# Da-Tsuchi/KLab_MultiModalModel

Measured on AMD Instinct MI355X. Metric: caption-train samples/sec (224px img, 64-tok tgt), higher is better.
Workload: dtype bf16; 1 GPU; BASELINE configs[1]: Swin-V2(C=64,(2,2,6,2),224,w7) frozen + T5-small, fwd+bwd+Adam, T5 dropout 0.1 on, random-init weights; global_batch=64, per_gpu_batch=64, src_len=9, tgt_len=64, parallelism=dp1, hipgraph=False, optimizer=klab.optim.FusedAdam (Adam update of ref/train.py:28, one kernel)

## Files before the change

### include/klab_mm.h

```cpp
#ifndef KLAB_MM_H
#define KLAB_MM_H
#include <stddef.h>
#include <stdint.h>

#ifdef __cplusplus
extern "C" {
#endif

#define KLAB_OK 0
#define KLAB_ERR_UNSUPPORTED (-2)
#define KLAB_ERR_BADARG (-3)

#define KLAB_F32 0
#define KLAB_BF16 1
#define KLAB_FP8 2

#define KLAB_ACT_NONE 0
#define KLAB_ACT_RELU 1
#define KLAB_ACT_GELU 2

#define KLAB_AUX_NONE 0
#define KLAB_AUX_NONZERO 1
#define KLAB_AUX_DGELU 2

// ... 77 lines not shown
int klab_t5_attn_fwd(const klab_attn_args* a, void* stream);
int klab_t5_attn_bwd(const klab_attn_args* a, void* stream);
typedef struct klab_attn_fused_args {
  const float* x; const float* gamma; float eps; int d_model;
  const void* w;
  void* xn; float* rstd;
  void* proj; long ldproj;
  int cross;
  klab_attn_args attn;
} klab_attn_fused_args;
int klab_t5_attn_fused_fwd(const klab_attn_fused_args* a, void* stream);
typedef struct klab_attn_bwd_fused_args {
  const void* dy; long lddy;
  const void* w;
  int d_model;
  klab_attn_args attn;
} klab_attn_bwd_fused_args;
int klab_t5_attn_bwd_fused(const klab_attn_bwd_fused_args* a, void* stream);
int klab_dbias_reduce(const void* ds_ws, int dtype, float* dbias, int nbatch, int H, int Lq, int Lk, void* stream);

typedef struct klab_swin_attn_args {
  int dtype;
  const void* qkv; void* ctx; const float* bias; const float* logit_scale; float* lse;
  int B, R, w, shift, H, C;
  const void* dctx; void* dqkv; float* dbias; float* dlogit_scale;
  void* bwd_ws; size_t bwd_ws_bytes;
  const float* bias_table; float* dbias_table;
  const float* v_bias; float* dv_bias;
} klab_swin_attn_args;
int klab_swin_attn_fwd(const klab_swin_attn_args* a, void* stream);
size_t klab_swin_attn_bwd_ws_bytes(int dtype, int B, int R, int w, int H, int C);
int klab_swin_qkv_attn_fused(const void* x, const void* wqkv, const float* bqkv, void* ctx, const float* bias, const float* logit_scale,
                             int dtype, int B, int R, int w, int shift, int H, int C, void* stream);
int klab_swin_attn_bwd(const klab_swin_attn_args* a, void* stream);
int klab_swin_cpb_bias(const float* coords, const int* index, const float* w0, const float* b0, const float* w2,
                       float* table, float* hidden, float* bias, int ntab, int n, int heads, int nhidden, void* stream);
int klab_swin_cpb_table(const float* coords, const float* w0, const float* b0, const float* w2, float* table, float* hidden,
                        float* bias_table, int ntab, int heads, int nhidden, void* stream);
int klab_swin_cpb_table_bwd(const float* dbias_table, const float* bias_table, const float* coords, const float* hidden, const float* w2,
                            float* dtable, float* dw0, float* db0, float* dw2, int ntab, int heads, int nhidden, void* stream);

typedef struct klab_image_desc { long long offset; int height, width; } klab_image_desc;
size_t klab_image_preprocess_ws_bytes(int n_images, int max_h, int mid);
int klab_image_preprocess(const unsigned char* src, const klab_image_desc* desc_dev, int n_images, int max_h, int max_w, int mid,
                          int out_size, int filter_a, int filter_b, double rescale, const float* mean3, const float* std3,
                          float* pixel_values, void* ws, size_t ws_bytes, void* stream);

#define KLAB_JPEG_GRAY 0
#define KLAB_JPEG_YCC 1
#define KLAB_JPEG_RGB 2
typedef struct klab_jpeg_info {
  int width, height, ncomp, precision, progressive, supported, colour;
  int hmax, vmax, mcus_x, mcus_y;
  int hs[3], vs[3], bw[3], bh[3], tq[3];
  long long coef_blocks;
} klab_jpeg_info;
typedef struct klab_jpeg_item { klab_jpeg_info info; long long coef_block0; long long rgb_off; } klab_jpeg_item;
int klab_jpeg_read_info(const unsigned char* data, size_t n, klab_jpeg_info* info);
int klab_jpeg_entropy_decode(const unsigned char* data, size_t n, short* coefs, unsigned short* qt, klab_jpeg_info* info);
int klab_jpeg_entropy_decode_batch(const unsigned char* const* data, const size_t* sizes, int n, short* const* coefs,
                                   unsigned short* qt, klab_jpeg_info* infos, int* rcs, int n_threads);
size_t klab_jpeg_decode_ws_bytes(const klab_jpeg_item* items, int n);
int klab_jpeg_decode_device(const short* coefs_dev, const unsigned short* qt_dev, const klab_jpeg_item* items,
                            const klab_jpeg_item* items_dev, int n, unsigned char* rgb_dev, void* ws, size_t ws_bytes, void* stream);

int klab_cast_pack(const void* desc_dev, int ndesc, long total4, void* dst, int dtype, void* stream);
// ... 204 lines not shown
```

### klab_multimodalmodel_amd/_lib.py

```python
import ctypes as C
import os

HERE = os.path.dirname(os.path.abspath(__file__))
LIB_PATH = os.environ.get("KLAB_LIB", os.path.join(HERE, "libklab_mm.so"))

F32, BF16, FP8 = 0, 1, 2
ACT_NONE, ACT_RELU, ACT_GELU = 0, 1, 2
AUX_NONE, AUX_NONZERO, AUX_DGELU = 0, 1, 2
ERR_UNSUPPORTED, ERR_BADARG = -2, -3

vp, i32, i64, f32, u32 = C.c_void_p, C.c_int, C.c_long, C.c_float, C.c_uint32


class GemmArgs(C.Structure):
    _fields_ = [("M", i32), ("N", i32), ("K", i32), ("dtype", i32),
                ("A", vp), ("lda", i64), ("a_kmajor", i32),
                ("B", vp), ("ldb", i64), ("b_kmajor", i32),
                ("C", vp), ("ldc", i64), ("c_dtype", i32), ("accumulate", i32),
                ("alpha", f32), ("alpha_dev", vp), ("bias", vp), ("act", i32),
                ("aux", vp), ("ldaux", i64), ("aux_mode", i32), ("aux_scale", f32),
                ("residual", vp), ("ldr", i64), ("r_dtype", i32),
                ("drop_p", f32), ("seed_dev", vp), ("drop_tag", u32), ("name_tag", i32), ("atomic_ok", i32)]


# ... 79 lines not shown
    "klab_layernorm_fwd": [vp, i32, vp, vp, vp, vp, vp, i32, vp, vp, i32, i32, f32, i32, i32, i32, f32, vp, u32, vp],
    "klab_layernorm_bwd": [vp, vp, i32, vp, vp, vp, vp, vp, vp, i32, i32, i32, i32, i32, f32, vp, u32, vp],
    "klab_rmsnorm_fwd_q8": [vp, vp, vp, vp, vp, vp, i32, i32, f32, f32, vp, u32, vp],
    "klab_layernorm_fwd_q8": [vp, vp, vp, vp, vp, vp, vp, vp, vp, vp, i32, i32, f32, vp],
    "klab_gelu_fwd": [vp, vp, i32, i64, vp],
    "klab_gelu_fwd_q8": [vp, vp, vp, vp, i32, i32, vp],
    "klab_geglu_fwd": [vp, i64, vp, i64, i32, i32, i32, f32, vp, u32, vp],
    "klab_geglu_bwd": [vp, i64, vp, i64, vp, i64, i32, i32, i32, f32, vp, u32, vp],
    "klab_layernorm_bwd_bias": [vp, vp, i32, vp, vp, vp, vp, vp, vp, vp, i32, i32, i32, i32, i32, f32, vp, u32, vp],
    "klab_t5_attn_fwd": [C.POINTER(AttnArgs), vp],
    "klab_t5_attn_bwd": [C.POINTER(AttnArgs), vp],
    "klab_t5_attn_fused_fwd": [C.POINTER(AttnFusedArgs), vp],
    "klab_t5_attn_bwd_fused": [C.POINTER(AttnBwdFusedArgs), vp],
    "klab_t5_beam_decode_attn": [i32, vp, i64, vp, vp, i64, i64, i32, vp, i64, vp, i64, vp, i64, i32, i32, i32, i32, vp],
    "klab_beam_topk": [i32, vp, i64, i32, vp, i32, i32, i32, vp, vp, vp, vp, vp],
    "klab_beam_update": [C.POINTER(BeamUpdateArgs), i32, vp],
    "klab_beam_init": [C.POINTER(BeamUpdateArgs), i32, i32, vp],
    "klab_beam_copy_rows": [i32, vp, i64, i32, vp, i64, i32, i32, vp],
    "klab_sample_rows": [C.POINTER(SampleArgs), vp],
    "klab_logits_process_rows": [C.POINTER(LogitsProcArgs), vp],
    "klab_gen_finalize": [vp, i64, vp, i64, i32, i32, i32, i32, f32, i32, vp, vp, vp, vp],
    "klab_sizeof_sample_args": [],
    "klab_sizeof_logits_proc_args": [],
    "klab_sizeof_gen_cfg": [],
    "klab_beam_topk_scores": [vp, i64, i32, vp, i32, i32, i32, vp, vp, vp, vp, vp],
    "klab_dbias_reduce": [vp, i32, vp, i32, i32, i32, i32, vp],
    "klab_swin_mlp_fused": [vp, vp, vp, vp, vp, vp, vp, vp, vp, vp, i32, i32, i32, f32, vp],
    "klab_gemm_grouped": [vp, i32, vp],
    "klab_gemm_grouped_tiles": [vp, i32, i32, vp],
    "klab_gemm_fp8": [C.POINTER(GemmArgs), vp, vp, i64, vp],
    "klab_quant_fp8_rows": [vp, i64, i32, i32, vp, i64, vp, vp],
    "klab_quant_fp8_arena": [vp, i32, i64, vp, vp, vp, vp],
    "klab_swin_qkv_attn_fused": [vp, vp, vp, vp, vp, vp, i32, i32, i32, i32, i32, i32, i32, vp],
    "klab_swin_linear_ln_fused": [vp, vp, vp, vp, vp, vp, vp, vp, i32, i32, i32, i32, f32, vp],
    "klab_swin_patch_embed_fused": [vp, vp, i32, vp, vp, vp, vp, vp, i32, i32, i32, i32, i32, i32, f32, vp],
    "klab_swin_proj_ln_fused": [vp, vp, vp, vp, vp, vp, vp, vp, i32, i32, i32, f32, vp],
    "klab_swin_attn_fwd": [C.POINTER(SwinAttnArgs), vp],
    "klab_swin_attn_bwd": [C.POINTER(SwinAttnArgs), vp],
    "klab_swin_attn_bwd_ws_bytes": [i32, i32, i32, i32, i32, i32],
    "klab_swin_cpb_bias": [vp, vp, vp, vp, vp, vp, vp, vp, i32, i32, i32, i32, vp],
    "klab_swin_cpb_table": [vp, vp, vp, vp, vp, vp, vp, i32, i32, i32, vp],
    "klab_swin_cpb_table_bwd": [vp, vp, vp, vp, vp, vp, vp, vp, vp, i32, i32, i32, vp],
    "klab_cast_pack": [vp, i32, i64, vp, i32, vp],
    "klab_embed_fwd": [vp, i32, i32, i32, i32, vp, i32, vp, i32, i32, f32, vp, u32, vp, vp],
    "klab_embed_bwd": [vp, i32, i32, i32, i32, vp, vp, i32, i32, i32, f32, vp, u32, vp],
    "klab_relbias_fwd": [vp, vp, vp, i32, i32, i32, vp],
    "klab_relbias_bwd": [vp, vp, vp, i32, i32, i32, i32, vp],
    "klab_ce_fwd": [vp, i64, i32, vp, i32, i32, vp, vp, vp, i32, vp],
    "klab_ce_count": [vp, i32, vp, vp],
    "klab_im2col_patch": [vp, vp, i32, i32, i32, i32, i32, vp],
    "klab_im2col_patch_ld": [vp, vp, i32, i32, i32, i32, i32, i32, vp],
    "klab_merge_gather": [vp, vp, i32, i32, i32, i32, vp],
    "klab_merge_scatter": [vp, vp, i32, i32, i32, vp],
    "klab_colsum": [vp, i64, i32, i32, i32, vp, vp],
    "klab_convert": [vp, vp, i32, i64, f32, vp],
    "klab_add_f32": [vp, vp, i64, vp],
    "klab_image_preprocess_ws_bytes": [i32, i32, i32],
    "klab_segv_trace_install": [i32],
    "klab_segv_set_context": [C.c_char_p],
    "klab_image_preprocess": [vp, vp, i32, i32, i32, i32, i32, i32, i32, C.c_double, vp, vp, vp, vp, C.c_size_t, vp],
    "klab_jpeg_read_info": [vp, C.c_size_t, vp],
    "klab_jpeg_entropy_decode": [vp, C.c_size_t, vp, vp, vp],
    "klab_jpeg_entropy_decode_batch": [vp, vp, i32, vp, vp, vp, vp, i32],
    "klab_jpeg_decode_ws_bytes": [vp, i32],
    "klab_jpeg_decode_device": [vp, vp, vp, vp, i32, vp, vp, C.c_size_t, vp],
}


class JpegInfo(C.Structure):
    _fields_ = [("width", i32), ("height", i32), ("ncomp", i32), ("precision", i32), ("progressive", i32), ("supported", i32),
                ("colour", i32), ("hmax", i32), ("vmax", i32), ("mcus_x", i32), ("mcus_y", i32), ("hs", i32 * 3), ("vs", i32 * 3),
                ("bw", i32 * 3), ("bh", i32 * 3), ("tq", i32 * 3), ("coef_blocks", C.c_longlong)]


class JpegItem(C.Structure):
    _fields_ = [("info", JpegInfo), ("coef_block0", C.c_longlong), ("rgb_off", C.c_longlong)]

_lib = None


class KlabError(RuntimeError):
    pass


def load():
    global _lib
    if _lib is not None:
        return _lib
    if not os.path.exists(LIB_PATH):
        raise KlabError(f"{LIB_PATH} is missing: run `python -m klab_multimodalmodel_amd.build` "
                        "(hipcc --offload-arch=gfx950). There is no CPU fallback.")
    import torch
    lib = C.CDLL(LIB_PATH)
    for name, argt in SIGNATURES.items():
        fn = getattr(lib, name)
        fn.argtypes = argt
        fn.restype = C.c_size_t if name.endswith("_ws_bytes") else i32
    _lib = lib
    return lib


def check(rc, what=""):
    if rc == 0:
        return
    if rc == ERR_UNSUPPORTED:
        raise NotImplementedError(f"klab: unsupported shape/alignment in {what}")
    if rc == ERR_BADARG:
        raise ValueError(f"klab: bad argument to {what}")
    raise KlabError(f"klab: {what} failed with hipError {rc}")


def ptr(t):
    return None if t is None else t.data_ptr()


def dtype_code(torch_dtype):
    import torch
    if torch_dtype == torch.float32:
        return F32
    if torch_dtype == torch.bfloat16:
        return BF16
    if torch_dtype == "fp8":
        return FP8
    raise ValueError(f"unsupported dtype {torch_dtype}")


def stream_ptr():
    import torch
    return torch.cuda.current_stream().cuda_stream
```

### klab_multimodalmodel_amd/csrc/attn_swin.hip

```cpp
#include <math.h>
#include <stdlib.h>
#include <string.h>

#include "common.h"
#include "klab_mm.h"

namespace klab {

struct SwinAttnP {
  const void* qkv; void* ctx; const float* bias; const float* logit_scale; float* lse;
  int B, R, w, shift, H, C;
  const void* dctx; void* dqkv; float* dbias; float* dlogit_scale;
};

__device__ __forceinline__ int swin_region(int s, int R, int w, int shift) { return (s >= R - w) + (s >= R - shift); }

template <typename T, int HD>
__global__ __launch_bounds__(64) void swin_attn_fwd_kernel(SwinAttnP p) {
  constexpr int VEC = Vec16<T>::N;
  constexpr int KST = HD + VEC;
  using V = typename Vec16<T>::type;
  extern __shared__ __attribute__((aligned(16))) char smem[];
  const int w = p.w, n = w * w, R = p.R, C = p.C, H = p.H;
  const int nWr = R / w, nW = nWr * nWr;
// ... 207 lines not shown
    const float inv = 1.f / sum;
    f32x4 o[2] = {f32x4{0.f, 0.f, 0.f, 0.f}, f32x4{0.f, 0.f, 0.f, 0.f}};
#pragma unroll
    for (int sidx = 0; sidx < 2; ++sidx) {
      const f32x4 a = st[2 * sidx], bb = st[2 * sidx + 1];
      const bf16x8 pf = {(bf16_t)(a[0] * inv), (bf16_t)(a[1] * inv), (bf16_t)(a[2] * inv), (bf16_t)(a[3] * inv),
                         (bf16_t)(bb[0] * inv), (bf16_t)(bb[1] * inv), (bf16_t)(bb[2] * inv), (bf16_t)(bb[3] * inv)};
      const int q4 = (lane & 15) >> 2, pp = lane & 3;
      const int r0 = sidx * 32 + 4 * g + q4;
#pragma unroll
      for (int dt = 0; dt < 2; ++dt) {
        const bf16x4 lo = __builtin_amdgcn_ds_read_tr16_b64_v4bf16((lds_bf16x4_sw*)(Vt + swin_tr_off(r0, dt * 16 + 4 * pp)));
        const bf16x4 hi = __builtin_amdgcn_ds_read_tr16_b64_v4bf16((lds_bf16x4_sw*)(Vt + swin_tr_off(r0 + 16, dt * 16 + 4 * pp)));
        const bf16x8 vf = {lo[0], lo[1], lo[2], lo[3], hi[0], hi[1], hi[2], hi[3]};
        o[dt] = __builtin_amdgcn_mfma_f32_16x16x32_bf16(vf, pf, o[dt], 0, 0, 0);
      }
    }
    if (q < n) {
#pragma unroll
      for (int dt = 0; dt < 2; ++dt)
        *reinterpret_cast<bf16x4*>(ctx + (long)tq * C + h * HD + dt * 16 + g * 4) =
            bf16x4{(bf16_t)o[dt][0], (bf16_t)o[dt][1], (bf16_t)o[dt][2], (bf16_t)o[dt][3]};
      if (g == 0 && p.lse) p.lse[(((long)b * nW + win) * H + h) * n + q] = m + __logf(sum);
    }
  }
}

struct SwinQkvP {
  const bf16_t* x; const bf16_t* wqkv; const float* bqkv;
  bf16_t* ctx; const float* bias; const float* logit_scale;
  int B, R, w, shift, H;
};

template <int C>
__global__ __launch_bounds__(64) void swin_qkv_attn_fused(SwinQkvP p) {
  constexpr int HD = 32, KP = 80, KB = C / 32;
  __shared__ __attribute__((aligned(16))) char Kr[64 * KP];
  __shared__ __attribute__((aligned(16))) char Vt[8 * 896];
  __shared__ int tok[64];
  __shared__ int reg[64];
  const int w = p.w, n = w * w, R = p.R, H = p.H;
  const int nWr = R / w, nW = nWr * nWr;
  const int lane = threadIdx.x, g = lane >> 4, lr = lane & 15;
  int bid = blockIdx.x;
  const int h = bid % H; bid /= H;
  const int win = bid % nW; const int b = bid / nW;
  const int wy = win / nWr, wx = win % nWr;
  {
    int t = 0, rg = -1;
    if (lane < n) {
      const int ys = wy * w + lane / w, xs = wx * w + lane % w;
      const int y = (ys + p.shift) % R, x = (xs + p.shift) % R;
      t = (b * R + y) * R + x;
      rg = p.shift > 0 ? swin_region(ys, R, w, p.shift) * 3 + swin_region(xs, R, w, p.shift) : 0;
    }
    tok[lane] = t; reg[lane] = rg;
  }
  __syncthreads();
  bf16x8 qh[4];
  auto finish_tile = [&](int mt, const f32x4 (&d)[6]) {
    const int j0 = mt * 16 + lr;
    float sq = 0.f, sk = 0.f;
#pragma unroll
    for (int r = 0; r < 4; ++r) { sq += d[0][r] * d[0][r] + d[1][r] * d[1][r]; sk += d[2][r] * d[2][r] + d[3][r] * d[3][r]; }
    sq += __shfl_xor(sq, 16, 64); sq += __shfl_xor(sq, 32, 64);
    sk += __shfl_xor(sk, 16, 64); sk += __shfl_xor(sk, 32, 64);
    const float iq = 1.f / fmaxf(sqrtf(sq), 1e-12f), ik = 1.f / fmaxf(sqrtf(sk), 1e-12f);
    qh[mt] = bf16x8{(bf16_t)(d[0][0] * iq), (bf16_t)(d[0][1] * iq), (bf16_t)(d[0][2] * iq), (bf16_t)(d[0][3] * iq),
                    (bf16_t)(d[1][0] * iq), (bf16_t)(d[1][1] * iq), (bf16_t)(d[1][2] * iq), (bf16_t)(d[1][3] * iq)};
    const bool valid = j0 < n;
#pragma unroll
    for (int hf = 0; hf < 2; ++hf) {
      const int col = hf * 16 + g * 4;
      bf16x4 kk = {(bf16_t)(d[2 + hf][0] * ik), (bf16_t)(d[2 + hf][1] * ik), (bf16_t)(d[2 + hf][2] * ik), (bf16_t)(d[2 + hf][3] * ik)};
      bf16x4 vv = {(bf16_t)d[4 + hf][0], (bf16_t)d[4 + hf][1], (bf16_t)d[4 + hf][2], (bf16_t)d[4 + hf][3]};
      if (!valid) { kk = bf16x4{}; vv = bf16x4{}; }
      *reinterpret_cast<bf16x4*>(Kr + j0 * KP + col * 2) = kk;
      *reinterpret_cast<bf16x4*>(Vt + swin_tr_off(j0, col)) = vv;
    }
  };
  f32x4 bq[6];
#pragma unroll
  for (int j = 0; j < 6; ++j) {
    const int row = (j >> 1) * C + h * HD + (j & 1) * 16;
    bq[j] = p.bqkv ? *reinterpret_cast<const f32x4*>(p.bqkv + row + g * 4) : f32x4{0.f, 0.f, 0.f, 0.f};
  }
  if constexpr (C <= 128) {
    bf16x8 wf[6][KB];
#pragma unroll
    for (int j = 0; j < 6; ++j) {
      const int row = (j >> 1) * C + h * HD + (j & 1) * 16;
#pragma unroll
      for (int kb = 0; kb < KB; ++kb) wf[j][kb] = *reinterpret_cast<const bf16x8*>(p.wqkv + (long)(row + lr) * C + kb * 32 + g * 8);
    }
    auto load_x = [&](int mt, bf16x8 (&xf)[KB]) {
      const int j0 = mt * 16 + lr;
      const int t = tok[j0 < n ? j0 : n - 1];
#pragma unroll
      for (int kb = 0; kb < KB; ++kb) xf[kb] = *reinterpret_cast<const bf16x8*>(p.x + (long)t * C + kb * 32 + g * 8);
    };
    bf16x8 xnext[KB];
    load_x(0, xnext);
#pragma unroll
    for (int mt = 0; mt < 4; ++mt) {
      bf16x8 xf[KB];
#pragma unroll
      for (int kb = 0; kb < KB; ++kb) xf[kb] = xnext[kb];
      if (mt + 1 < 4) load_x(mt + 1, xnext);
      f32x4 d[6];
#pragma unroll
      for (int j = 0; j < 6; ++j) {
        d[j] = bq[j];
#pragma unroll
        for (int kb = 0; kb < KB; ++kb) d[j] = __builtin_amdgcn_mfma_f32_16x16x32_bf16(wf[j][kb], xf[kb], d[j], 0, 0, 0);
      }
      finish_tile(mt, d);
    }
  } else {
    const long trow[4] = {(long)tok[min(lr, n - 1)] * C, (long)tok[min(16 + lr, n - 1)] * C, (long)tok[min(32 + lr, n - 1)] * C,
                          (long)tok[min(48 + lr, n - 1)] * C};
    auto load_kb = [&](int kb, bf16x8 (&wf)[6], bf16x8 (&xf)[4]) {
#pragma unroll
      for (int j = 0; j < 6; ++j)
        wf[j] = *reinterpret_cast<const bf16x8*>(p.wqkv + (long)((j >> 1) * C + h * HD + (j & 1) * 16 + lr) * C + kb * 32 + g * 8);
#pragma unroll
      for (int mt = 0; mt < 4; ++mt) xf[mt] = *reinterpret_cast<const bf16x8*>(p.x + trow[mt] + kb * 32 + g * 8);
    };
    f32x4 d[4][6];
#pragma unroll
    for (int mt = 0; mt < 4; ++mt)
#pragma unroll
      for (int j = 0; j < 6; ++j) d[mt][j] = bq[j];
    bf16x8 wn[6], xn[4];
    load_kb(0, wn, xn);
    for (int kb = 0; kb < KB; ++kb) {
      bf16x8 wc[6], xc[4];
#pragma unroll
      for (int j = 0; j < 6; ++j) wc[j] = wn[j];
#pragma unroll
      for (int mt = 0; mt < 4; ++mt) xc[mt] = xn[mt];
      if (kb + 1 < KB) load_kb(kb + 1, wn, xn);
#pragma unroll
      for (int mt = 0; mt < 4; ++mt)
#pragma unroll
        for (int j = 0; j < 6; ++j) d[mt][j] = __builtin_amdgcn_mfma_f32_16x16x32_bf16(wc[j], xc[mt], d[mt][j], 0, 0, 0);
    }
#pragma unroll
    for (int mt = 0; mt < 4; ++mt) finish_tile(mt, d[mt]);
  }
  __syncthreads();
  const float scale = __expf(fminf(p.logit_scale[h], 4.6051701859880914f));
  auto fetch_bias = [&](int qt, f32x4 (&bv)[4]) {
    const int q = qt * 16 + lr;
    const float* brow = p.bias + ((long)h * n + (q < n ? q : n - 1)) * n;
#pragma unroll
    for (int t = 0; t < 4; ++t)
#pragma unroll
      for (int r = 0; r < 4; ++r) { const int key = t * 16 + g * 4 + r; bv[t][r] = brow[key < n ? key : n - 1]; }
  };
  const int nqt = (n + 15) / 16;
  f32x4 bnext[4];
  fetch_bias(0, bnext);
#pragma unroll
  for (int qt = 0; qt < 4; ++qt) {
    if (qt >= nqt) break;
    const int q = qt * 16 + lr;
    const int qc = q < n ? q : n - 1;
    const int tq = tok[qc], rq = reg[qc];
    f32x4 bcur[4] = {bnext[0], bnext[1], bnext[2], bnext[3]};
    if (qt + 1 < nqt) fetch_bias(qt + 1, bnext);
    f32x4 st[4];
    float m = -INFINITY;
#pragma unroll
    for (int t = 0; t < 4; ++t) {
      const char* krow = Kr + (t * 16 + lr) * KP;
      const bf16x4 lo = *reinterpret_cast<const bf16x4*>(krow + g * 8), hi = *reinterpret_cast<const bf16x4*>(krow + 32 + g * 8);
      const bf16x8 kf = {lo[0], lo[1], lo[2], lo[3], hi[0], hi[1], hi[2], hi[3]};
      st[t] = __builtin_amdgcn_mfma_f32_16x16x32_bf16(kf, qh[qt], f32x4{0.f, 0.f, 0.f, 0.f}, 0, 0, 0);
#pragma unroll
      for (int r = 0; r < 4; ++r) {
        const int key = t * 16 + g * 4 + r;
        float x = st[t][r] * scale + bcur[t][r] + (reg[key] != rq ? -200.f : 0.f);
        x = key < n ? x : -INFINITY;
        st[t][r] = x;
        m = fmaxf(m, x);
      }
    }
    m = fmaxf(m, __shfl_xor(m, 16, 64));
    m = fmaxf(m, __shfl_xor(m, 32, 64));
    float sum = 0.f;
#pragma unroll
    for (int t = 0; t < 4; ++t)
#pragma unroll
      for (int r = 0; r < 4; ++r) { const float e = __expf(st[t][r] - m); st[t][r] = e; sum += e; }
    sum += __shfl_xor(sum, 16, 64);
    sum += __shfl_xor(sum, 32, 64);
    const float inv = 1.f / sum;
    f32x4 o[2] = {f32x4{0.f, 0.f, 0.f, 0.f}, f32x4{0.f, 0.f, 0.f, 0.f}};
#pragma unroll
    for (int sidx = 0; sidx < 2; ++sidx) {
      const f32x4 a = st[2 * sidx], bb = st[2 * sidx + 1];
      const bf16x8 pf = {(bf16_t)(a[0] * inv), (bf16_t)(a[1] * inv), (bf16_t)(a[2] * inv), (bf16_t)(a[3] * inv),
                         (bf16_t)(bb[0] * inv), (bf16_t)(bb[1] * inv), (bf16_t)(bb[2] * inv), (bf16_t)(bb[3] * inv)};
      const int q4 = lr >> 2, pp = lane & 3;
      const int r0 = sidx * 32 + 4 * g + q4;
#pragma unroll
      for (int dt = 0; dt < 2; ++dt) {
        const bf16x4 lo = __builtin_amdgcn_ds_read_tr16_b64_v4bf16((lds_bf16x4_sw*)(Vt + swin_tr_off(r0, dt * 16 + 4 * pp)));
        const bf16x4 hi = __builtin_amdgcn_ds_read_tr16_b64_v4bf16((lds_bf16x4_sw*)(Vt + swin_tr_off(r0 + 16, dt * 16 + 4 * pp)));
        const bf16x8 vf = {lo[0], lo[1], lo[2], lo[3], hi[0], hi[1], hi[2], hi[3]};
        o[dt] = __builtin_amdgcn_mfma_f32_16x16x32_bf16(vf, pf, o[dt], 0, 0, 0);
      }
    }
    if (q < n) {
#pragma unroll
      for (int dt = 0; dt < 2; ++dt)
        *reinterpret_cast<bf16x4*>(p.ctx + (long)tq * C + h * HD + dt * 16 + g * 4) =
            bf16x4{(bf16_t)o[dt][0], (bf16_t)o[dt][1], (bf16_t)o[dt][2], (bf16_t)o[dt][3]};
    }
  }
}

template <typename T, int HD>
__global__ __launch_bounds__(64) void swin_attn_bwd_kernel(SwinAttnP p) {
  constexpr int VEC = Vec16<T>::N;
  constexpr int KST = HD + VEC;
  using V = typename Vec16<T>::type;
  extern __shared__ __attribute__((aligned(16))) char smem[];
  const int w = p.w, n = w * w, R = p.R, C = p.C, H = p.H;
  const int nWr = R / w, nW = nWr * nWr;
  T* Kn = reinterpret_cast<T*>(smem);
  T* Vs = Kn + (size_t)n * KST;
  float* dKn = reinterpret_cast<float*>(Vs + (size_t)n * KST);
  float* dVs = dKn + (size_t)n * HD;
  float* kinv = dVs + (size_t)n * HD;
  int* tok = reinterpret_cast<int*>(kinv + n);
  int* reg = tok + n;
  const int lane = threadIdx.x;
  int bid = blockIdx.x;
  const int h = bid % H; bid /= H;
  const int win = bid % nW; const int b = bid / nW;
  const int wy = win / nWr, wx = win % nWr;
  const T* qkv = reinterpret_cast<const T*>(p.qkv);
  const T* dctx = reinterpret_cast<const T*>(p.dctx);
  T* dqkv = reinterpret_cast<T*>(p.dqkv);
  const long ld = 3L * C;

  for (int j = lane; j < n; j += 64) {
    const int ys = wy * w + j / w, xs = wx * w + j % w;
    const int y = (ys + p.shift) % R, x = (xs + p.shift) % R;
    const int t = (b * R + y) * R + x;
    tok[j] = t;
    reg[j] = p.shift > 0 ? swin_region(ys, R, w, p.shift) * 3 + swin_region(xs, R, w, p.shift) : 0;
// ... 605 lines not shown
  }
  const long tot = (long)heads * n * n;
  hipLaunchKernelGGL(cpb_dtable_kernel, dim3((unsigned)((tot + 255) / 256)), dim3(256), 0, s, dbias, bias, index, dtable, heads, n * n);
  KLAB_LAUNCH_CHECK();
  if (ntab > 192)
    return cpb_mlp_bwd_any_launch(dtable, coords, hidden, w2, dw0, db0, dw2, ntab, heads, nhidden, s);
  const size_t cpb_lds = ((size_t)ntab * heads + (size_t)(heads > 3 ? heads : 3) * 16 * 17) * 4;
  if (cpb_lds > 64 * 1024) return KLAB_ERR_UNSUPPORTED;
  hipLaunchKernelGGL(cpb_mlp_bwd_kernel, dim3((nhidden + 15) / 16), dim3(256), cpb_lds, s, dtable, coords, hidden, w2, dw0, db0, dw2, ntab, heads, nhidden);
  KLAB_LAUNCH_CHECK();
  return KLAB_OK;
}

extern "C" int klab_swin_cpb_bias_bwd(const float* dbias, const float* bias, const int* index, const float* coords, const float* hidden,
                                      const float* w0, const float* w2, float* dtable, float* dw0, float* db0, float* dw2, int ntab, int n,
                                      int heads, int nhidden, void* stream) {
  return klab_swin_cpb_bias_bwd_pz(dbias, bias, index, coords, hidden, w0, w2, dtable, dw0, db0, dw2, ntab, n, heads, nhidden, 0, stream);
}

extern "C" int klab_swin_qkv_attn_fused(const void* x, const void* wqkv, const float* bqkv, void* ctx, const float* bias, const float* logit_scale,
                                        int dtype, int B, int R, int w, int shift, int H, int C, void* stream) {
  if (!x || !wqkv || !ctx || !bias || !logit_scale || B <= 0 || R <= 0 || w <= 0 || H <= 0) return KLAB_ERR_BADARG;
  if (dtype != KLAB_BF16 || C != H * 32 || w * w > 64 || R % w || shift < 0 || shift >= w) return KLAB_ERR_UNSUPPORTED;
  SwinQkvP p{(const bf16_t*)x, (const bf16_t*)wqkv, bqkv, (bf16_t*)ctx, bias, logit_scale, B, R, w, shift, H};
  const int nW = (R / w) * (R / w);
  hipStream_t s = (hipStream_t)stream;
  if (C == 64) hipLaunchKernelGGL(swin_qkv_attn_fused<64>, dim3(B * nW * H), dim3(64), 0, s, p);
  else if (C == 128) hipLaunchKernelGGL(swin_qkv_attn_fused<128>, dim3(B * nW * H), dim3(64), 0, s, p);
  else if (C == 256) hipLaunchKernelGGL(swin_qkv_attn_fused<256>, dim3(B * nW * H), dim3(64), 0, s, p);
  else return KLAB_ERR_UNSUPPORTED;
  KLAB_LAUNCH_CHECK();
  return KLAB_OK;
}
```

### klab_multimodalmodel_amd/csrc/engine.cpp

```cpp
#include <hip/hip_runtime.h>
#include <math.h>
#include <stdio.h>
#include <string.h>

#include <string>
#include <vector>

#include "gemm_shared.h"
#include "klab_mm.h"

namespace {

#define RC(x)                 \
  do {                        \
    int rc__ = (x);           \
    if (rc__ != 0) return rc__; \
  } while (0)

struct ParamInfo {
  std::string name;
  std::vector<long> shape;
  long numel = 0;
  long grad_off = -1;
  long warena_off = -1;
  long farena_off = -1;
};

struct T5LayerIdx { int q, k, v, o, relb, ln0, cq, ck, cv, co, ln1, wi, wi1, wo, ln2; };
struct T5Idx { int shared, lm_head = -1, head = -1; std::vector<T5LayerIdx> enc, dec; int enc_final, dec_final; };
struct SwinBlockIdx { int ls, c0w, c0b, c2w, qw, qb, kw, vw, vb, pw, pb, ln1w, ln1b, f1w, f1b, f2w, f2b, ln2w, ln2b; };
struct SwinStageIdx { std::vector<SwinBlockIdx> blk; int redw, mnw, mnb; };
struct SwinIdx { int pew, peb, penw, penb; std::vector<SwinStageIdx> st; int lnw, lnb; };

struct T5LayerBufs {
  void *xn1, *qkv, *ctx; float *lse, *rstd1;
  void *xn2, *qc, *ctx2; float *lse2, *rstd2;
  void *xn3, *hmid; float* rstd3;
  void* ab;
};
struct T5StackBufs {
  std::vector<float*> h;
  std::vector<T5LayerBufs> L;
  void* out_t = nullptr; float* rstd_f = nullptr;
  float* bias = nullptr; float* dbias = nullptr; const int* bucket = nullptr;
  int M = 0, Lseq = 0;
};
struct SwinBlockBufs {
  float* x_in; void* xt_in;
  void *qkv, *ctx, *po; float *lse, *mean1, *rstd1; float* h1; void* h1t;
  void *z, *a, *fo; float *mean2, *rstd2; float* h2; void* h2t;
  float *bias, *table, *hidden;
  float* btab;
  int R, w, shift, H, C; long M;
};
struct SwinStageBufs { std::vector<SwinBlockBufs> blk; void *mg, *mo; float *mmean, *mrstd; float* xm; void* xmt; };

struct Bump {
  char* base; size_t off = 0;
  explicit Bump(void* b) : base((char*)b) {}
  void* take(size_t bytes) {
    off = (off + 255) & ~(size_t)255;
    void* p = base ? base + off : nullptr;
    off += bytes;
    return p;
  }
};

struct ProcSet {
  bool on = false;
  klab_logits_proc_cfg cfg{1.f};
  std::vector<int> table;
};
struct GenRun {
  klab_gen_cfg cfg{};
  ProcSet lp;
  int cur = 0;
};

}

struct klab_engine {
  klab_model_cfg cfg;
  std::vector<ParamInfo> P[3];
  SwinIdx si; T5Idx li, mi;
  long grad_elems[3] = {0, 0, 0};
// ... 406 lines not shown
  const long T0 = (long)R0 * R0, M0 = (long)B * T0, K0 = (long)s.in_ch * s.patch * s.patch, C0 = s.embed_dim;
  e->cols = b.take((size_t)M0 * ((K0 + 31) & ~31L) * es);
  e->pe_out = b.take((size_t)M0 * C0 * es);
  e->pe_mean = (float*)b.take((size_t)M0 * 4); e->pe_rstd = (float*)b.take((size_t)M0 * 4);
  e->x0 = (float*)b.take((size_t)M0 * C0 * 4); e->x0t = b.take((size_t)M0 * C0 * es);
  e->sw.assign(s.n_stages, SwinStageBufs());
  long maxMC = M0 * C0;
  for (int st = 0; st < s.n_stages; ++st) {
    const int R = R0 >> st;
    const long C = C0 << st, M = (long)B * R * R, F = (long)s.mlp_ratio * C;
    const int H = s.heads[st];
    const int w = R < s.window ? R : s.window;
    const int nWr = (R + (w > 0 ? w : 1) - 1) / (w > 0 ? w : 1);
    const int n = w * w, nW = nWr * nWr;
    const int ntab = (2 * w - 1) * (2 * w - 1);
    if (M * C > maxMC) maxMC = M * C;
    SwinStageBufs& sb = e->sw[st];
    sb.blk.resize(s.depths[st]);
    for (int k = 0; k < s.depths[st]; ++k) {
      SwinBlockBufs& q = sb.blk[k];
      q.R = R; q.w = w; q.H = H; q.C = (int)C; q.M = M;
      q.shift = (k % 2 == 0 || R <= w) ? 0 : s.window / 2;
      q.qkv = b.take((size_t)M * 3 * C * es); q.ctx = b.take((size_t)M * C * es); q.po = b.take((size_t)M * C * es);
      q.lse = (float*)b.take((size_t)B * nW * H * n * 4);
      q.mean1 = (float*)b.take((size_t)M * 4); q.rstd1 = (float*)b.take((size_t)M * 4);
      q.h1 = (float*)b.take((size_t)M * C * 4); q.h1t = b.take((size_t)M * C * es);
      q.z = c.train_swin ? b.take((size_t)M * F * es) : nullptr;
      q.a = b.take((size_t)M * F * es); q.fo = b.take((size_t)M * C * es);
      q.mean2 = (float*)b.take((size_t)M * 4); q.rstd2 = (float*)b.take((size_t)M * 4);
      q.h2 = (float*)b.take((size_t)M * C * 4); q.h2t = b.take((size_t)M * C * es);
      const bool big = n > 64 || (R % w) != 0;
      q.bias = big ? nullptr : (float*)b.take((size_t)H * n * n * 4);
      q.btab = big ? (float*)b.take((size_t)ntab * H * 4) : nullptr;
      q.table = (float*)b.take((size_t)ntab * H * 4);
      q.hidden = (float*)b.take((size_t)ntab * 512 * 4);
    }
    sb.mg = sb.mo = nullptr; sb.mmean = sb.mrstd = nullptr; sb.xm = nullptr; sb.xmt = nullptr;
    if (st < s.n_stages - 1) {
      const long M2 = M / 4;
      sb.mg = b.take((size_t)M2 * 4 * C * es); sb.mo = b.take((size_t)M2 * 2 * C * es);
      sb.mmean = (float*)b.take((size_t)M2 * 4); sb.mrstd = (float*)b.take((size_t)M2 * 4);
      sb.xm = (float*)b.take((size_t)M2 * 2 * C * 4); sb.xmt = b.take((size_t)M2 * 2 * C * es);
    }
  }
  const long Ml = (long)B * Nimg;
  e->sw_fmean = (float*)b.take((size_t)Ml * 4); e->sw_frstd = (float*)b.take((size_t)Ml * 4);
  if (c.train_swin) {
    const long F0 = (long)s.mlp_ratio;
    e->sdh_a = (float*)b.take((size_t)maxMC * 4); e->sdh_b = (float*)b.take((size_t)maxMC * 4);
    e->sdm = (float*)b.take((size_t)maxMC * 4);
    e->sdy = b.take((size_t)maxMC * es); e->sdctx = b.take((size_t)maxMC * es);
    e->sdqkv = b.take((size_t)maxMC * 3 * es); e->sda = b.take((size_t)maxMC * F0 * es);
    for (int pz = 0; pz < 2; ++pz) {
      e->sdyA[pz] = b.take((size_t)maxMC * es); e->sdyB[pz] = b.take((size_t)maxMC * es);
      e->sdaP[pz] = b.take((size_t)maxMC * F0 * es); e->sdqkvP[pz] = b.take((size_t)maxMC * 3 * es);
    }
    int maxn = 0, maxH = 0, maxn_small = 1;
    for (int st = 0; st < s.n_stages; ++st) {
      const int R = R0 >> st; const int w = R < s.window ? R : s.window;
      if (w * w > maxn) maxn = w * w;
      if (w * w <= 64 && w * w > maxn_small) maxn_small = w * w;
      if (s.heads[st] > maxH) maxH = s.heads[st];
    }
    int nblk = 0;
    for (int st = 0; st < s.n_stages; ++st) nblk += s.depths[st];
    e->sdb_stride = ((long)maxH * maxn_small * maxn_small + 63) & ~63L;
// ... 443 lines not shown
  static const bool fused_pe = klab::env_on("KLAB_SWIN_FUSED_EMBED");
  int perc = KLAB_ERR_UNSUPPORTED;
  if (!e->cfg.train_swin && fused_pe && !e->fp8 && Kp >= 64)
    perc = klab_swin_patch_embed_fused(pixels, woff(c, P[e->si.pew].warena_off), Kp, W[e->si.peb], W[e->si.penw], W[e->si.penb], e->x0, e->x0t, c.dt,
                                       B, s.in_ch, s.image_size, s.patch, C0, s.ln_eps, c.ws());
  if (perc != 0 && perc != KLAB_ERR_UNSUPPORTED) return perc;
  if (perc != 0) {
  RC(klab_im2col_patch_ld(pixels, e->cols, c.dt, B, s.in_ch, s.image_size, s.patch, Kp, c.ws()));
  {
    klab_gemm_args g = G0(c, (int)M0, C0, Kp, e->cols, Kp, 1, woff(c, P[e->si.pew].warena_off), Kp, 1, e->pe_out, C0, c.dt);
    g.bias = W[e->si.peb];
    RC(klab_gemm(&g, c.ws()));
  }
  RC(klab_layernorm_fwd(e->pe_out, c.dt, W[e->si.penw], W[e->si.penb], nullptr, e->x0, e->x0t, c.dt, e->pe_mean, e->pe_rstd, (int)M0, C0,
                        s.ln_eps, 0, 0, 0, 0.f, nullptr, 0, c.ws()));
  }
  float* x = e->x0;
  void* xt = e->x0t;
  long bias_off = 0;
  for (int st = 0; st < s.n_stages; ++st) {
    SwinStageBufs& sb = e->sw[st];
    for (size_t k = 0; k < sb.blk.size(); ++k) {
      SwinBlockBufs& q = sb.blk[k];
      const SwinBlockIdx& ix = e->si.st[st].blk[k];
      const int C = q.C, M = (int)q.M, F = s.mlp_ratio * C, n = q.w * q.w;
      q.x_in = x; q.xt_in = xt;
      if (refresh_bias) {
        if (q.btab)
          RC(klab_swin_cpb_table(e->swin_coords[st], W[ix.c0w], W[ix.c0b], W[ix.c2w], q.table, q.hidden, q.btab, e->swin_ntab[st], q.H, 512,
                                 c.ws()));
        else
          RC(klab_swin_cpb_bias(e->swin_coords[st], e->swin_index[st], W[ix.c0w], W[ix.c0b], W[ix.c2w], q.table, q.hidden, q.bias,
                                e->swin_ntab[st], n, q.H, 512, c.ws()));
      }
      const float* qkvb = ix.qb >= 0 ? e->farena + bias_off : nullptr;
      bias_off += 3 * C;
      int qrc = KLAB_ERR_UNSUPPORTED;
      if (!e->cfg.train_swin && q.bias)
        qrc = klab_swin_qkv_attn_fused(xt, woff(c, P[ix.qw].warena_off), qkvb, q.ctx, q.bias, W[ix.ls], c.dt, B, q.R, q.w, q.shift, q.H, C,
                                       c.ws());
      if (qrc != 0 && qrc != KLAB_ERR_UNSUPPORTED) return qrc;
      if (qrc != 0) {
        RC(linear_fwd(c, xt, M, C, P[ix.qw].warena_off, 3 * C, q.qkv, 3 * C, c.dt, qkvb));
        klab_swin_attn_args a;
        memset(&a, 0, sizeof(a));
        a.dtype = c.dt; a.qkv = q.qkv; a.ctx = q.ctx; a.bias = q.bias; a.bias_table = q.btab; a.logit_scale = W[ix.ls]; a.lse = q.lse;
        a.B = B; a.R = q.R; a.w = q.w; a.shift = q.shift; a.H = q.H; a.C = C;
        a.bwd_ws = e->sattn_ws; a.bwd_ws_bytes = e->sattn_ws_bytes;
        a.v_bias = qkvb ? qkvb + 2 * C : nullptr;
        RC(klab_swin_attn_fwd(&a, c.ws()));
      }
      int prc = KLAB_ERR_UNSUPPORTED;
      if (!e->cfg.train_swin)
        prc = klab_swin_proj_ln_fused(q.ctx, x, woff(c, P[ix.pw].warena_off), W[ix.pb], W[ix.ln1w], W[ix.ln1b], q.h1, q.h1t, c.dt, M, C, s.ln_eps,
                                      c.ws());
      if (prc != 0 && prc != KLAB_ERR_UNSUPPORTED) return prc;
      static const bool fused_lin_ln = klab::env_on("KLAB_SWIN_FUSED_LIN_LN");
      const bool wide_ln = !e->cfg.train_swin && !e->fp8 && fused_lin_ln;
      if (prc != 0 && wide_ln) {
        prc = klab_swin_linear_ln_fused(q.ctx, x, woff(c, P[ix.pw].warena_off), W[ix.pb], W[ix.ln1w], W[ix.ln1b], q.h1, q.h1t, c.dt, M, C, C,
                                        s.ln_eps, c.ws());
        if (prc != 0 && prc != KLAB_ERR_UNSUPPORTED) return prc;
      }
      if (prc != 0) {
        RC(linear_fwd(c, q.ctx, M, C, P[ix.pw].warena_off, C, q.po, C, c.dt, W[ix.pb]));
        RC(ln_fwd_for_linear(c, q.po, W[ix.ln1w], W[ix.ln1b], x, q.h1, q.h1t, q.mean1, q.rstd1, M, C, s.ln_eps));
      }
      if (e->cfg.train_swin) {
        RC(linear_fwd(c, q.h1t, M, C, P[ix.f1w].warena_off, F, q.z, F, c.dt, W[ix.f1b]));
        RC(gelu_fwd_for_linear(c, q.z, q.a, M, F));
      } else {
// ... 1202 lines not shown
```

### klab_multimodalmodel_amd/ops.py

```python
import ctypes as C

import torch

from . import _lib as L


def _seed_ptr(seed):
    return None if seed is None else seed.data_ptr()


def _gemm_args(A, B, C_out, *, M, N, K, a_kmajor=True, b_kmajor=True, lda=None, ldb=None, ldc=None, alpha=1.0,
               alpha_dev=None, bias=None, act=L.ACT_NONE, aux=None, aux_mode=L.AUX_NONE, aux_scale=1.0, residual=None,
               drop_p=0.0, seed=None, tag=0, accumulate=False, atomic_ok=False, name_tag=0):
    a = L.GemmArgs()
    a.atomic_ok, a.name_tag = int(atomic_ok), name_tag
    a.M, a.N, a.K = M, N, K
    a.dtype = L.dtype_code(A.dtype)
    assert B.dtype == A.dtype
    a.A, a.lda, a.a_kmajor = A.data_ptr(), (lda if lda is not None else A.stride(0)), int(a_kmajor)
    a.B, a.ldb, a.b_kmajor = B.data_ptr(), (ldb if ldb is not None else B.stride(0)), int(b_kmajor)
    a.C, a.ldc, a.c_dtype = C_out.data_ptr(), (ldc if ldc is not None else C_out.stride(0)), L.dtype_code(C_out.dtype)
    a.accumulate = int(accumulate)
    a.alpha = alpha
    a.alpha_dev = L.ptr(alpha_dev)
# ... 78 lines not shown


def rmsnorm_bwd_part(dy, x, w, rstd, dw_part, dres=None, dx=None, dxt=None, grp=0, grp_stride=0, off=0, p_y=0.0, tag_y=0,
                     p_prev=0.0, tag_prev=0, seed=None):
    lib = L.load()
    rows, d = x.shape
    L.check(lib.klab_rmsnorm_bwd_part(dy.data_ptr(), x.data_ptr(), w.data_ptr(), rstd.data_ptr(), L.ptr(dres), L.ptr(dx), L.ptr(dxt),
                                      L.dtype_code(dxt.dtype) if dxt is not None else 0, dw_part.data_ptr(), rows, d, grp, grp_stride,
                                      off, p_y, tag_y, p_prev, tag_prev, _seed_ptr(seed), L.stream_ptr()), "klab_rmsnorm_bwd_part")


def colpart_reduce(part, call_stride, nparts, d, dsts):
    lib = L.load()
    table = torch.tensor([t.data_ptr() for t in dsts], dtype=torch.int64).to(part.device)
    L.check(lib.klab_colpart_reduce(part.data_ptr(), int(call_stride), int(nparts), int(d), table.data_ptr(), len(dsts), L.stream_ptr()),
            "klab_colpart_reduce")
    return table


def layernorm_fwd(y, gamma, beta, shortcut=None, out=None, outt=None, mean=None, rstd=None, eps=1e-5, grp=0, grp_stride=0,
                  off=0, drop_p=0.0, seed=None, tag=0):
    lib = L.load()
    rows, Cc = y.shape
    L.check(lib.klab_layernorm_fwd(y.data_ptr(), L.dtype_code(y.dtype), gamma.data_ptr(), beta.data_ptr(), L.ptr(shortcut),
                                   L.ptr(out), L.ptr(outt), L.dtype_code(outt.dtype) if outt is not None else 0, L.ptr(mean),
                                   L.ptr(rstd), rows, Cc, eps, grp, grp_stride, off, drop_p, _seed_ptr(seed), tag,
                                   L.stream_ptr()), "klab_layernorm_fwd")


def swin_qkv_attn_fused(x, wqkv, bqkv, ctx, bias, logit_scale, *, B, R, w, shift, H, C):
    lib = L.load()
    L.check(lib.klab_swin_qkv_attn_fused(x.data_ptr(), wqkv.data_ptr(), L.ptr(bqkv), ctx.data_ptr(), bias.data_ptr(), logit_scale.data_ptr(),
                                         L.dtype_code(x.dtype), B, R, w, shift, H, C, L.stream_ptr()), "klab_swin_qkv_attn_fused")


def swin_proj_ln_fused(x, shortcut, w, b, gamma, beta, out, outt=None, eps=1e-5):
    lib = L.load()
    M, Cc = x.shape
    L.check(lib.klab_swin_proj_ln_fused(x.data_ptr(), shortcut.data_ptr(), w.data_ptr(), b.data_ptr(), gamma.data_ptr(), beta.data_ptr(),
                                        out.data_ptr(), L.ptr(outt), L.dtype_code(x.dtype), M, Cc, eps, L.stream_ptr()), "klab_swin_proj_ln_fused")


def swin_mlp_fused(x, shortcut, w1, b1, w2, b2, gamma, beta, out, outt=None, eps=1e-5):
    lib = L.load()
    M, Cc = x.shape
    L.check(lib.klab_swin_mlp_fused(x.data_ptr(), shortcut.data_ptr(), w1.data_ptr(), b1.data_ptr(), w2.data_ptr(), b2.data_ptr(),
                                    gamma.data_ptr(), beta.data_ptr(), out.data_ptr(), L.ptr(outt), L.dtype_code(x.dtype), M, Cc, eps,
                                    L.stream_ptr()), "klab_swin_mlp_fused")


def rmsnorm_fwd_q8(x, w, y, rstd, y8, yscale, eps=1e-6):
    lib = L.load()
    rows, d = x.shape
    L.check(lib.klab_rmsnorm_fwd_q8(x.data_ptr(), w.data_ptr(), y.data_ptr(), L.ptr(rstd), y8.data_ptr(), yscale.data_ptr(), rows, d, eps, 0.0,
                                    None, 0, L.stream_ptr()), "klab_rmsnorm_fwd_q8")


def layernorm_fwd_q8(y, gamma, beta, shortcut, out, outt, mean, rstd, o8, oscale, eps=1e-5):
    lib = L.load()
    rows, Cc = y.shape
    L.check(lib.klab_layernorm_fwd_q8(y.data_ptr(), gamma.data_ptr(), beta.data_ptr(), L.ptr(shortcut), L.ptr(out), outt.data_ptr(), L.ptr(mean),
                                      L.ptr(rstd), o8.data_ptr(), oscale.data_ptr(), rows, Cc, eps, L.stream_ptr()), "klab_layernorm_fwd_q8")


def gelu_fwd(z, a):
    lib = L.load()
# ... 433 lines not shown
```

Before: 11690 samples/s.

## Precompute Swin attention bias+mask images in MFMA-fragment layout for fused QKV-attn

Adds a kernel that precomputes, per head and window class (edge/corner for shifted windows), the relative-position bias plus shift mask and padding -inf, laid out exactly in the MFMA fragment order. A new fused QKV-attention variant loads that image with vectorized f32x4 reads instead of gathering per-key bias, comparing region ids and masking per element. It also adds occupancy launch bounds and sched barriers. This removes scalar gathers and mask arithmetic from the inner softmax loop, at the cost of a small extra kernel per block and extra workspace.

```diff
diff --git a/include/klab_mm.h b/include/klab_mm.h
--- a/include/klab_mm.h
+++ b/include/klab_mm.h
@@ -133,6 +133,10 @@
 size_t klab_swin_attn_bwd_ws_bytes(int dtype, int B, int R, int w, int H, int C);
 int klab_swin_qkv_attn_fused(const void* x, const void* wqkv, const float* bqkv, void* ctx, const float* bias, const float* logit_scale,
                              int dtype, int B, int R, int w, int shift, int H, int C, void* stream);
+size_t klab_swin_bias_image_bytes(int w, int shift, int H);
+int klab_swin_bias_image(const float* bias, float* image, int R, int w, int shift, int H, void* stream);
+int klab_swin_qkv_attn_fused_img(const void* x, const void* wqkv, const float* bqkv, void* ctx, const float* image, const float* logit_scale,
+                                 int dtype, int B, int R, int w, int shift, int H, int C, void* stream);
 int klab_swin_attn_bwd(const klab_swin_attn_args* a, void* stream);
 int klab_swin_cpb_bias(const float* coords, const int* index, const float* w0, const float* b0, const float* w2,
                        float* table, float* hidden, float* bias, int ntab, int n, int heads, int nhidden, void* stream);
diff --git a/klab_multimodalmodel_amd/_lib.py b/klab_multimodalmodel_amd/_lib.py
--- a/klab_multimodalmodel_amd/_lib.py
+++ b/klab_multimodalmodel_amd/_lib.py
@@ -135,6 +135,9 @@
     "klab_quant_fp8_rows": [vp, i64, i32, i32, vp, i64, vp, vp],
     "klab_quant_fp8_arena": [vp, i32, i64, vp, vp, vp, vp],
     "klab_swin_qkv_attn_fused": [vp, vp, vp, vp, vp, vp, i32, i32, i32, i32, i32, i32, i32, vp],
+    "klab_swin_bias_image_bytes": [i32, i32, i32],
+    "klab_swin_bias_image": [vp, vp, i32, i32, i32, i32, vp],
+    "klab_swin_qkv_attn_fused_img": [vp, vp, vp, vp, vp, vp, i32, i32, i32, i32, i32, i32, i32, vp],
     "klab_swin_linear_ln_fused": [vp, vp, vp, vp, vp, vp, vp, vp, i32, i32, i32, i32, f32, vp],
     "klab_swin_patch_embed_fused": [vp, vp, i32, vp, vp, vp, vp, vp, i32, i32, i32, i32, i32, i32, f32, vp],
     "klab_swin_proj_ln_fused": [vp, vp, vp, vp, vp, vp, vp, vp, i32, i32, i32, f32, vp],
@@ -198,7 +201,7 @@
     for name, argt in SIGNATURES.items():
         fn = getattr(lib, name)
         fn.argtypes = argt
-        fn.restype = C.c_size_t if name.endswith("_ws_bytes") else i32
+        fn.restype = C.c_size_t if name.endswith("_bytes") else i32
     _lib = lib
     return lib
 
diff --git a/klab_multimodalmodel_amd/csrc/attn_swin.hip b/klab_multimodalmodel_amd/csrc/attn_swin.hip
--- a/klab_multimodalmodel_amd/csrc/attn_swin.hip
+++ b/klab_multimodalmodel_amd/csrc/attn_swin.hip
@@ -263,13 +263,13 @@
   int B, R, w, shift, H;
 };
 
-template <int C>
-__global__ __launch_bounds__(64) void swin_qkv_attn_fused(SwinQkvP p) {
+template <int C, bool IMG>
+__device__ __forceinline__ void swin_qkv_attn_body(const SwinQkvP& p) {
   constexpr int HD = 32, KP = 80, KB = C / 32;
   __shared__ __attribute__((aligned(16))) char Kr[64 * KP];
   __shared__ __attribute__((aligned(16))) char Vt[8 * 896];
   __shared__ int tok[64];
-  __shared__ int reg[64];
+  __shared__ int reg[IMG ? 1 : 64];
   const int w = p.w, n = w * w, R = p.R, H = p.H;
   const int nWr = R / w, nW = nWr * nWr;
   const int lane = threadIdx.x, g = lane >> 4, lr = lane & 15;
@@ -285,7 +285,8 @@
       t = (b * R + y) * R + x;
       rg = p.shift > 0 ? swin_region(ys, R, w, p.shift) * 3 + swin_region(xs, R, w, p.shift) : 0;
     }
-    tok[lane] = t; reg[lane] = rg;
+    tok[lane] = t;
+    if constexpr (!IMG) reg[lane] = rg;
   }
   __syncthreads();
   bf16x8 qh[4];
@@ -334,6 +335,7 @@
     load_x(0, xnext);
 #pragma unroll
     for (int mt = 0; mt < 4; ++mt) {
+      if constexpr (IMG) __builtin_amdgcn_sched_barrier(0);
       bf16x8 xf[KB];
 #pragma unroll
       for (int kb = 0; kb < KB; ++kb) xf[kb] = xnext[kb];
@@ -381,13 +383,20 @@
   }
   __syncthreads();
   const float scale = __expf(fminf(p.logit_scale[h], 4.6051701859880914f));
+  const int cls = IMG && p.shift > 0 ? (wy == nWr - 1) * 2 + (wx == nWr - 1) : 0;
   auto fetch_bias = [&](int qt, f32x4 (&bv)[4]) {
-    const int q = qt * 16 + lr;
-    const float* brow = p.bias + ((long)h * n + (q < n ? q : n - 1)) * n;
-#pragma unroll
-    for (int t = 0; t < 4; ++t)
-#pragma unroll
-      for (int r = 0; r < 4; ++r) { const int key = t * 16 + g * 4 + r; bv[t][r] = brow[key < n ? key : n - 1]; }
+    if constexpr (IMG) {
+      const float* ip = p.bias + ((((long)cls * H + h) * 4 + qt) * 64 + lane) * 16;
+#pragma unroll
+      for (int t = 0; t < 4; ++t) bv[t] = *reinterpret_cast<const f32x4*>(ip + t * 4);
+    } else {
+      const int q = qt * 16 + lr;
+      const float* brow = p.bias + ((long)h * n + (q < n ? q : n - 1)) * n;
+#pragma unroll
+      for (int t = 0; t < 4; ++t)
+#pragma unroll
+        for (int r = 0; r < 4; ++r) { const int key = t * 16 + g * 4 + r; bv[t][r] = brow[key < n ? key : n - 1]; }
+    }
   };
   const int nqt = (n + 15) / 16;
   f32x4 bnext[4];
@@ -397,7 +406,8 @@
     if (qt >= nqt) break;
     const int q = qt * 16 + lr;
     const int qc = q < n ? q : n - 1;
-    const int tq = tok[qc], rq = reg[qc];
+    if constexpr (IMG) __builtin_amdgcn_sched_barrier(0);
+    const int tq = tok[qc], rq = IMG ? 0 : reg[qc];
     f32x4 bcur[4] = {bnext[0], bnext[1], bnext[2], bnext[3]};
     if (qt + 1 < nqt) fetch_bias(qt + 1, bnext);
     f32x4 st[4];
@@ -410,9 +420,14 @@
       st[t] = __builtin_amdgcn_mfma_f32_16x16x32_bf16(kf, qh[qt], f32x4{0.f, 0.f, 0.f, 0.f}, 0, 0, 0);
 #pragma unroll
       for (int r = 0; r < 4; ++r) {
-        const int key = t * 16 + g * 4 + r;
-        float x = st[t][r] * scale + bcur[t][r] + (reg[key] != rq ? -200.f : 0.f);
-        x = key < n ? x : -INFINITY;
+        float x;
+        if constexpr (IMG) {
+          x = fmaf(st[t][r], scale, bcur[t][r]);
+        } else {
+          const int key = t * 16 + g * 4 + r;
+          x = st[t][r] * scale + bcur[t][r] + (reg[key] != rq ? -200.f : 0.f);
+          x = key < n ? x : -INFINITY;
+        }
         st[t][r] = x;
         m = fmaxf(m, x);
       }
@@ -450,6 +465,31 @@
             bf16x4{(bf16_t)o[dt][0], (bf16_t)o[dt][1], (bf16_t)o[dt][2], (bf16_t)o[dt][3]};
     }
   }
+}
+
+template <int C>
+__global__ __launch_bounds__(64) void swin_qkv_attn_fused(SwinQkvP p) { swin_qkv_attn_body<C, false>(p); }
+
+template <int C>
+__global__ __launch_bounds__(64, C <= 64 ? 3 : 2) void swin_qkv_attn_fused_img(SwinQkvP p) { swin_qkv_attn_body<C, true>(p); }
+
+__global__ __launch_bounds__(256) void swin_bias_image_kernel(const float* __restrict__ bias, float* __restrict__ image, int R, int w, int shift,
+                                                              int H, int total) {
+  const int i = blockIdx.x * 256 + threadIdx.x;
+  if (i >= total) return;
+  const int n = w * w;
+  const int r = i & 3, t = (i >> 2) & 3, lane = (i >> 4) & 63, qt = (i >> 10) & 3;
+  const int h = (i >> 12) % H, cls = (i >> 12) / H;
+  const int q = qt * 16 + (lane & 15), key = t * 16 + (lane >> 4) * 4 + r;
+  const int qc = q < n ? q : n - 1, kc = key < n ? key : n - 1;
+  const int y0 = (cls & 2) ? R - w : 0, x0 = (cls & 1) ? R - w : 0;
+  int rq = 0, rk = 0;
+  if (shift > 0) {
+    rq = ((cls & 2) ? swin_region(y0 + qc / w, R, w, shift) : 0) * 3 + ((cls & 1) ? swin_region(x0 + qc % w, R, w, shift) : 0);
+    rk = ((cls & 2) ? swin_region(y0 + kc / w, R, w, shift) : 0) * 3 + ((cls & 1) ? swin_region(x0 + kc % w, R, w, shift) : 0);
+  }
+  const float b = bias[((long)h * n + qc) * n + kc];
+  image[i] = key < n ? (rq != rk ? b + -200.f : b) : -INFINITY;
 }
 
 template <typename T, int HD>
@@ -1121,3 +1161,32 @@
   KLAB_LAUNCH_CHECK();
   return KLAB_OK;
 }
+
+extern "C" size_t klab_swin_bias_image_bytes(int w, int shift, int H) {
+  if (w <= 0 || w * w > 64 || H <= 0 || shift < 0) return 0;
+  return (size_t)(shift > 0 ? 4 : 1) * H * 4 * 64 * 16 * sizeof(float);
+}
+
+extern "C" int klab_swin_bias_image(const float* bias, float* image, int R, int w, int shift, int H, void* stream) {
+  if (!bias || !image || R <= 0 || w <= 0 || H <= 0) return KLAB_ERR_BADARG;
+  if (w * w > 64 || R % w || shift < 0 || shift >= w) return KLAB_ERR_UNSUPPORTED;
+  const int total = (int)(klab_swin_bias_image_bytes(w, shift, H) / sizeof(float));
+  hipLaunchKernelGGL(swin_bias_image_kernel, dim3((total + 255) / 256), dim3(256), 0, (hipStream_t)stream, bias, image, R, w, shift, H, total);
+  KLAB_LAUNCH_CHECK();
+  return KLAB_OK;
+}
+
+extern "C" int klab_swin_qkv_attn_fused_img(const void* x, const void* wqkv, const float* bqkv, void* ctx, const float* image,
+                                            const float* logit_scale, int dtype, int B, int R, int w, int shift, int H, int C, void* stream) {
+  if (!x || !wqkv || !ctx || !image || !logit_scale || B <= 0 || R <= 0 || w <= 0 || H <= 0) return KLAB_ERR_BADARG;
+  if (dtype != KLAB_BF16 || C != H * 32 || w * w > 64 || R % w || shift < 0 || shift >= w) return KLAB_ERR_UNSUPPORTED;
+  SwinQkvP p{(const bf16_t*)x, (const bf16_t*)wqkv, bqkv, (bf16_t*)ctx, image, logit_scale, B, R, w, shift, H};
+  const int nW = (R / w) * (R / w);
+  hipStream_t s = (hipStream_t)stream;
+  if (C == 64) hipLaunchKernelGGL(swin_qkv_attn_fused_img<64>, dim3(B * nW * H), dim3(64), 0, s, p);
+  else if (C == 128) hipLaunchKernelGGL(swin_qkv_attn_fused_img<128>, dim3(B * nW * H), dim3(64), 0, s, p);
+  else if (C == 256) hipLaunchKernelGGL(swin_qkv_attn_fused_img<256>, dim3(B * nW * H), dim3(64), 0, s, p);
+  else return KLAB_ERR_UNSUPPORTED;
+  KLAB_LAUNCH_CHECK();
+  return KLAB_OK;
+}
diff --git a/klab_multimodalmodel_amd/csrc/engine.cpp b/klab_multimodalmodel_amd/csrc/engine.cpp
--- a/klab_multimodalmodel_amd/csrc/engine.cpp
+++ b/klab_multimodalmodel_amd/csrc/engine.cpp
@@ -45,12 +45,14 @@
   float* bias = nullptr; float* dbias = nullptr; const int* bucket = nullptr;
   int M = 0, Lseq = 0;
 };
+inline bool swin_attn_on_image(int C) { return C == 64 || C == 128 || C == 256; }
 struct SwinBlockBufs {
   float* x_in; void* xt_in;
   void *qkv, *ctx, *po; float *lse, *mean1, *rstd1; float* h1; void* h1t;
   void *z, *a, *fo; float *mean2, *rstd2; float* h2; void* h2t;
   float *bias, *table, *hidden;
   float* btab;
+  float* bimg;
   int R, w, shift, H, C; long M;
 };
 struct SwinStageBufs { std::vector<SwinBlockBufs> blk; void *mg, *mo; float *mmean, *mrstd; float* xm; void* xmt; };
@@ -523,6 +525,7 @@
       const bool big = n > 64 || (R % w) != 0;
       q.bias = big ? nullptr : (float*)b.take((size_t)H * n * n * 4);
       q.btab = big ? (float*)b.take((size_t)ntab * H * 4) : nullptr;
+      q.bimg = (!big && !c.train_swin && swin_attn_on_image((int)C)) ? (float*)b.take(klab_swin_bias_image_bytes(w, q.shift, H)) : nullptr;
       q.table = (float*)b.take((size_t)ntab * H * 4);
       q.hidden = (float*)b.take((size_t)ntab * 512 * 4);
     }
@@ -1032,11 +1035,15 @@
         else
           RC(klab_swin_cpb_bias(e->swin_coords[st], e->swin_index[st], W[ix.c0w], W[ix.c0b], W[ix.c2w], q.table, q.hidden, q.bias,
                                 e->swin_ntab[st], n, q.H, 512, c.ws()));
+        if (q.bimg) RC(klab_swin_bias_image(q.bias, q.bimg, q.R, q.w, q.shift, q.H, c.ws()));
       }
       const float* qkvb = ix.qb >= 0 ? e->farena + bias_off : nullptr;
       bias_off += 3 * C;
       int qrc = KLAB_ERR_UNSUPPORTED;
-      if (!e->cfg.train_swin && q.bias)
+      if (q.bimg)
+        qrc = klab_swin_qkv_attn_fused_img(xt, woff(c, P[ix.qw].warena_off), qkvb, q.ctx, q.bimg, W[ix.ls], c.dt, B, q.R, q.w, q.shift, q.H, C,
+                                           c.ws());
+      else if (!e->cfg.train_swin && q.bias)
         qrc = klab_swin_qkv_attn_fused(xt, woff(c, P[ix.qw].warena_off), qkvb, q.ctx, q.bias, W[ix.ls], c.dt, B, q.R, q.w, q.shift, q.H, C,
                                        c.ws());
       if (qrc != 0 && qrc != KLAB_ERR_UNSUPPORTED) return qrc;
diff --git a/klab_multimodalmodel_amd/ops.py b/klab_multimodalmodel_amd/ops.py
--- a/klab_multimodalmodel_amd/ops.py
+++ b/klab_multimodalmodel_amd/ops.py
@@ -134,6 +134,25 @@
     lib = L.load()
     L.check(lib.klab_swin_qkv_attn_fused(x.data_ptr(), wqkv.data_ptr(), L.ptr(bqkv), ctx.data_ptr(), bias.data_ptr(), logit_scale.data_ptr(),
                                          L.dtype_code(x.dtype), B, R, w, shift, H, C, L.stream_ptr()), "klab_swin_qkv_attn_fused")
+
+
+def swin_bias_image(bias, *, R, w, shift):
+    import torch
+    lib = L.load()
+    H = bias.shape[0]
+    nbytes = lib.klab_swin_bias_image_bytes(w, shift, H)
+    if nbytes == 0:
+        raise NotImplementedError("klab: unsupported shape/alignment in klab_swin_bias_image_bytes")
+    image = torch.empty(nbytes // (H * 4 * 64 * 16 * 4), H, 4, 64, 16, device=bias.device, dtype=torch.float32)
+    L.check(lib.klab_swin_bias_image(bias.data_ptr(), image.data_ptr(), R, w, shift, H, L.stream_ptr()), "klab_swin_bias_image")
+    return image
+
+
+def swin_qkv_attn_fused_img(x, wqkv, bqkv, ctx, image, logit_scale, *, B, R, w, shift, H, C):
+    lib = L.load()
+    L.check(lib.klab_swin_qkv_attn_fused_img(x.data_ptr(), wqkv.data_ptr(), L.ptr(bqkv), ctx.data_ptr(), image.data_ptr(),
+                                             logit_scale.data_ptr(), L.dtype_code(x.dtype), B, R, w, shift, H, C, L.stream_ptr()),
+            "klab_swin_qkv_attn_fused_img")
 
 
 def swin_proj_ln_fused(x, shortcut, w, b, gamma, beta, out, outt=None, eps=1e-5):
```

Result: faster. 11850 samples/s (median of 6 runs) (+1.3%).
